# ryancinsight/imaginary

Hardware: AMD Instinct MI355X
Metric: images/sec (4K RGB->1080p Lanczos3 batch) + achieved HBM GB/s, 1/2/4/8 GPUs (higher is better)
Workload: dtype u8; 1 GPU; C2: batched 3840x2160x3 -> 1920x1080x3 Lanczos3 reduce (bimg /resize?width=1920&height=1080), corner sampling convention (PARITY_ASSUMPTIONS.md row 1), k_reduce2x2; batch_per_gpu=256, global_batch=256, parallelism=dp1 (independent shards)

## Files before the change

### imaginary_amd/csrc/k_reduce.hip

```cpp
#include <hip/hip_runtime.h>

#include <algorithm>
#include <cmath>
#include <cstdlib>
#include <vector>

#include "device_common.h"

namespace mipx {
namespace {

using namespace dev;

constexpr int kR = 12;
template <int WIDE, int TIGHT = 0>
struct R2T {
    static constexpr int kThreads = 128 << WIDE;
    static constexpr int kPitch = WIDE == 2 ? 544 : WIDE == 1 ? (TIGHT ? 264 : 288) : 160;
};

template <int B, int WIDE = 0, int TIGHT = 0>
struct R2 {
    static constexpr int kThreads = R2T<WIDE, TIGHT>::kThreads;
    static constexpr int kPitch = R2T<WIDE, TIGHT>::kPitch;
    static constexpr int TW = B == 3 ? 80 << WIDE : WIDE == 0 ? 56 : 60 << WIDE;
    static constexpr int NPX = 2 * TW + 9;
    static constexpr int K = B == 3 ? 4 : 2;
    static constexpr int OFF0 = B == 3 ? 1 : 0;
    static constexpr int ND = (B * NPX + OFF0 + 3) / 4;
    static_assert(ND <= kThreads && ND <= kPitch, "strip too wide");
    static_assert(((TW / K) * K) == TW, "items must tile the strip");
    static_assert((B * 2 * K) % 8 == 0, "window start must be 8-byte aligned");
};

struct Reduce2Args {
    const u8 *in;
    u8 *out;
    int w, h, ow, oh;
    int n_strips, n_bands, band_rows;
    int s_base, y_base, x_end, y_end;
    long long in_img, out_img;
    float c0, c1, c3, c5, bias;
    int remap;
    int band_major;
};

typedef float f2v __attribute__((ext_vector_type(2)));
typedef float f4v __attribute__((ext_vector_type(4)));

__device__ __forceinline__ f4v cvt4_once(uint32_t v) {
    return f4v{ubyte_once<0>(v), ubyte_once<1>(v), ubyte_once<2>(v), ubyte_once<3>(v)};
}
__device__ __forceinline__ f2v lo2(f4v v) { return __builtin_shufflevector(v, v, 0, 1); }
__device__ __forceinline__ f2v hi2(f4v v) { return __builtin_shufflevector(v, v, 2, 3); }

__device__ __forceinline__ float tap7(float c0, float c1, float c3, float c5, float bias, float e, float m1,
                                      float p1, float m3, float p3, float m5, float p5) {
    float acc = __builtin_fmaf(c0, e, bias);
    acc = __builtin_fmaf(c1, m1 + p1, acc);
    acc = __builtin_fmaf(c3, m3 + p3, acc);
    return __builtin_fmaf(c5, m5 + p5, acc);
}
__device__ __forceinline__ f2v tap7v(f2v c0, f2v c1, f2v c3, f2v c5, f2v bias, f2v e, f2v m1, f2v p1, f2v m3,
                                     f2v p3, f2v m5, f2v p5) {
    f2v acc = __builtin_elementwise_fma(c0, e, bias);
    acc = __builtin_elementwise_fma(c1, m1 + p1, acc);
    acc = __builtin_elementwise_fma(c3, m3 + p3, acc);
    return __builtin_elementwise_fma(c5, m5 + p5, acc);
}
__device__ __forceinline__ uint32_t pack4b(float a, float b, float c, float d) {
    uint32_t v = __builtin_amdgcn_cvt_pk_u8_f32(a, 0, 0u);
    v = __builtin_amdgcn_cvt_pk_u8_f32(b, 1, v);
    v = __builtin_amdgcn_cvt_pk_u8_f32(c, 2, v);
    return __builtin_amdgcn_cvt_pk_u8_f32(d, 3, v);
}

template <int B, int R, bool PF, bool PK, bool MEM, int LAUX, bool NTS, int WIDE, int TIGHT>
__device__ __forceinline__ void reduce2_tile(const Reduce2Args &a, int img, int strip, int band,
                                             uint32_t *lds) {
    using G = R2<B, WIDE, TIGHT>;
    constexpr int kThreads = G::kThreads, kPitch = G::kPitch;
    constexpr int TW = G::TW, K = G::K;
    const int tid = threadIdx.x;
    const int x0 = (a.s_base + strip) * TW;
    const int row_bytes = a.w * B;
    const int px0 = 2 * x0 - 5;
    const int base = (B * px0) & ~3;
    const int byte0 = base + 4 * tid;
    const bool vlane = tid < G::ND && byte0 >= 0 && byte0 + 4 <= row_bytes;
    const __amdgpu_buffer_rsrc_t rsrc = __builtin_amdgcn_make_buffer_rsrc(
        const_cast<u8 *>(a.in + img * a.in_img), 0, static_cast<int>(a.in_img), 0x00020000);
    const uint32_t voff = vlane ? static_cast<uint32_t>(byte0) : 0x80000000u;
    const int y0 = a.y_base + band * a.band_rows;
    const int y1 = min(y0 + a.band_rows, a.y_end);
    const float c0 = a.c0, c1 = a.c1, c3 = a.c3, c5 = a.c5, bias = a.bias;
    const int nl = px0 < 0 ? -px0 : 0;
    const int x_last = min(x0 + TW, a.x_end) - 1;
    const int fr = a.w - px0;
    const int fr_end = min(2 * x_last + 5 - px0, G::NPX - 1);
    const int nr = fr_end >= fr ? fr_end - fr + 1 : 0;
    const bool edge = nl > 0 || nr > 0;

    auto load_row = [&](int r) -> uint32_t {
        r = clampi(r, 0, a.h - 1);
        return static_cast<uint32_t>(__builtin_amdgcn_raw_buffer_load_b32(rsrc, voff, r * row_bytes, LAUX));
    };

    f4v ring[6];
    ring[3] = cvt4_once(load_row(2 * (y0 - 3) + 1));
    ring[4] = cvt4_once(load_row(2 * (y0 - 2) + 1));
    ring[5] = cvt4_once(load_row(2 * (y0 - 1) + 1));
    ring[0] = cvt4_once(load_row(2 * y0 + 1));
    ring[1] = cvt4_once(load_row(2 * (y0 + 1) + 1));
    ring[2] = f4v{0.f, 0.f, 0.f, 0.f};

    uint32_t odd[R], even[R];
    if (PF) {
#pragma unroll
        for (int u = 0; u < R; ++u) {
            odd[u] = load_row(2 * (y0 + u + 2) + 1);
            even[u] = load_row(2 * (y0 + u));
        }
    }
    int buf = 0;
    for (int yc = y0; yc < y1; yc += R, buf ^= 1) {
        uint32_t *L = lds + buf * (R * kPitch);
        if (!PF) {
#pragma unroll
            for (int u = 0; u < R; ++u) {
                odd[u] = load_row(2 * (yc + u + 2) + 1);
                even[u] = load_row(2 * (yc + u));
            }
        }
        const bool more = yc + R < y1;
#pragma unroll
        for (int u = 0; u < R; ++u) {
            uint32_t d;
            if (MEM) {
                d = odd[u] + even[u];
                if (PF && more) {
                    odd[u] = load_row(2 * (yc + R + u + 2) + 1);
                    even[u] = load_row(2 * (yc + R + u));
                }
            } else {
                ring[(u + 2) % 6] = cvt4_once(odd[u]);
                const f4v e = cvt4_once(even[u]);
                if (PF && more) {
                    odd[u] = load_row(2 * (yc + R + u + 2) + 1);
                    even[u] = load_row(2 * (yc + R + u));
                }
                const f4v m5 = ring[(u + 3) % 6], m3 = ring[(u + 4) % 6], m1 = ring[(u + 5) % 6];
                const f4v p1 = ring[u % 6], p3 = ring[(u + 1) % 6], p5 = ring[(u + 2) % 6];
                if (PK) {
                    const f2v C0 = {c0, c0}, C1 = {c1, c1}, C3 = {c3, c3}, C5 = {c5, c5}, BI = {bias, bias};
                    const f2v a = tap7v(C0, C1, C3, C5, BI, lo2(e), lo2(m1), lo2(p1), lo2(m3), lo2(p3), lo2(m5),
                                        lo2(p5));
                    const f2v b = tap7v(C0, C1, C3, C5, BI, hi2(e), hi2(m1), hi2(p1), hi2(m3), hi2(p3), hi2(m5),
                                        hi2(p5));
                    d = pack4b(a.x, a.y, b.x, b.y);
                } else {
                    d = pack4b(tap7(c0, c1, c3, c5, bias, e.x, m1.x, p1.x, m3.x, p3.x, m5.x, p5.x),
                               tap7(c0, c1, c3, c5, bias, e.y, m1.y, p1.y, m3.y, p3.y, m5.y, p5.y),
                               tap7(c0, c1, c3, c5, bias, e.z, m1.z, p1.z, m3.z, p3.z, m5.z, p5.z),
                               tap7(c0, c1, c3, c5, bias, e.w, m1.w, p1.w, m3.w, p3.w, m5.w, p5.w));
                }
            }
            if (G::ND >= kThreads || tid < G::ND) L[u * kPitch + tid] = d;
        }
        if (edge) {
            __syncthreads();
            u8 *Lb = reinterpret_cast<u8 *>(L);
            const int nfill = nl + nr;
            for (int i = tid; i < R * nfill * B; i += kThreads) {
                const int u = i / (nfill * B);
                const int rem = i - u * nfill * B;
                const int f = rem / B, c = rem - f * B;
                const int dst = f < nl ? f : fr + (f - nl);
                const int srcp = f < nl ? nl : fr - 1;
                Lb[u * kPitch * 4 + B * dst + G::OFF0 + c] = Lb[u * kPitch * 4 + B * srcp + G::OFF0 + c];
            }
        }
        __syncthreads();
        constexpr int items_per_row = TW / K;
        for (int it = tid; it < R * items_per_row; it += kThreads) {
            const int u = it / items_per_row;
            const int j = it - u * items_per_row;
            const int x = x0 + K * j;
            const int y = yc + u;
            if (y >= a.y_end || x >= a.x_end) continue;
            const uint32_t *row = L + u * kPitch;
            constexpr int W0 = (B * 2 * K) / 4;
            uint32_t win[13];
            if (B == 3) {
                const uint2 *r2 = reinterpret_cast<const uint2 *>(row + W0 * j);
#pragma unroll
                for (int q = 0; q < 6; ++q) {
                    const uint2 dd = r2[q];
                    win[2 * q] = dd.x;
                    win[2 * q + 1] = dd.y;
                }
                win[12] = row[W0 * j + 12];
            } else {
                const uint4 *r4 = reinterpret_cast<const uint4 *>(row + W0 * j);
#pragma unroll
                for (int q = 0; q < 3; ++q) {
                    const uint4 dd = r4[q];
                    win[4 * q] = dd.x, win[4 * q + 1] = dd.y, win[4 * q + 2] = dd.z, win[4 * q + 3] = dd.w;
                }
                win[12] = row[W0 * j + 12];
            }
            float o[K][B];
            if (MEM) {
#pragma unroll
                for (int k = 0; k < K; ++k)
#pragma unroll
                    for (int c = 0; c < B; ++c) o[k][c] = __uint_as_float(win[(k * B + c) % 13] & 0x437f0000u);
            } else
#pragma unroll
            for (int c = 0; c < B; ++c) {
                float px[2 * K + 9];
#pragma unroll
                for (int t = 0; t < 2 * K + 9; ++t) {
                    const int lb = B * t + c + G::OFF0;
                    const uint32_t dd = win[lb >> 2];
                    switch (lb & 3) {
                        case 0: px[t] = ubyte_once<0>(dd); break;
                        case 1: px[t] = ubyte_once<1>(dd); break;
                        case 2: px[t] = ubyte_once<2>(dd); break;
                        default: px[t] = ubyte_once<3>(dd); break;
                    }
                }
#pragma unroll
                for (int k = 0; k < K; ++k) {
                    const int m = 2 * k + 5;
                    o[k][c] = tap7(c0, c1, c3, c5, bias, px[m], px[m - 1], px[m + 1], px[m - 3], px[m + 3],
                                   px[m - 5], px[m + 5]);
                }
            }
            u8 *q = a.out + img * a.out_img + (static_cast<size_t>(y) * a.ow + x) * B;
            const bool full = x + K <= a.ow;
            if (B == 3) {
                const uint32_t d0 = pack4b(o[0][0], o[0][1], o[0][2], o[1][0]);
                const uint32_t d1 = pack4b(o[1][1], o[1][2], o[2][0], o[2][1]);
                const uint32_t d2 = pack4b(o[2][2], o[3][0], o[3][1], o[3][2]);
                if (full && (reinterpret_cast<uintptr_t>(q) & 3u) == 0) {
                    if (NTS) {
                        typedef uint32_t u3v __attribute__((ext_vector_type(3)));
                        __builtin_nontemporal_store(u3v{d0, d1, d2}, reinterpret_cast<u3v *>(q));
                    } else {
                        *reinterpret_cast<uint3 *>(q) = uint3{d0, d1, d2};
                    }
                } else {
                    const uint32_t dd[3] = {d0, d1, d2};
                    const int nb = (full ? K : a.ow - x) * B;
                    for (int i = 0; i < nb; ++i) q[i] = static_cast<u8>(dd[i >> 2] >> (8 * (i & 3)));
                }
            } else {
                const uint32_t d0 = pack4b(o[0][0], o[0][1], o[0][2], o[0][3]);
                const uint32_t d1 = pack4b(o[1][0], o[1][1], o[1][2], o[1][3]);
                uint32_t *q32 = reinterpret_cast<uint32_t *>(q);
                if (full && (reinterpret_cast<uintptr_t>(q) & 7u) == 0) {
                    *reinterpret_cast<uint2 *>(q) = uint2{d0, d1};
                } else {
                    q32[0] = d0;
                    if (full) q32[1] = d1;
                }
            }
        }
    }
}


template <int B, int VAR>
__global__ void __launch_bounds__(R2T<(VAR & 128) ? 2 : (VAR & 64) ? 1 : 0>::kThreads) k_reduce2x2(Reduce2Args a) {
    constexpr int WIDE = (VAR & 128) ? 2 : (VAR & 64) ? 1 : 0;
    constexpr int TIGHT = (VAR & 256) ? 1 : 0;
    constexpr int kPitch = R2T<WIDE, TIGHT>::kPitch;
    constexpr int R = (VAR & 1) ? 6 : 12;
    constexpr bool PF = (VAR & 2) != 0;
    constexpr bool PK = (VAR & 4) != 0;
    constexpr bool MEM = (VAR & 8) != 0;
    constexpr int LAUX = (VAR & 16) ? 2 : 0;
    constexpr bool NTS = (VAR & 32) != 0;
    __shared__ uint32_t lds[2 * R * kPitch];
    const uint32_t t = a.remap ? xcd_remap(blockIdx.x, gridDim.x) : blockIdx.x;
    int strip, band, img;
    if (a.band_major) {
        band = t % a.n_bands;
        const int rest = t / a.n_bands;
        strip = rest % a.n_strips;
        img = rest / a.n_strips;
    } else {
        strip = t % a.n_strips;
        const int rest = t / a.n_strips;
        band = rest % a.n_bands;
        img = rest / a.n_bands;
    }
    reduce2_tile<B, R, PF, PK, MEM, LAUX, NTS, WIDE, TIGHT>(a, img, strip, band, lds);
}


}

int reducev_launch(const u8 *in, u8 *out, int n, int w, int h, int b, double vshrink, hipStream_t st) {
    SepSpec spec;
    if (!sep_spec_reduce(vshrink, &spec)) return MIPX_EDEVICE;
    SepWindow win{};
    win.bands = b;
    win.in_pitch = w * b;
    win.in_base = 0;
    win.in_img = img_bytes(w, h, b);
    win.in_len = h;
    win.o0 = 0;
    win.out_w = w;
    win.out_h = out_size_reduce(h, vshrink);
    return vpass_launch(in, out, n, spec, win, st);
}

int reduceh_launch(const u8 *in, u8 *out, int n, int w, int h, int b, double hshrink, hipStream_t st) {
    SepSpec spec;
    if (!sep_spec_reduce(hshrink, &spec)) return MIPX_EDEVICE;
    SepWindow win{};
    win.bands = b;
    win.in_pitch = w * b;
    win.in_base = 0;
    win.in_img = img_bytes(w, h, b);
    win.in_len = w;
    win.o0 = 0;
    win.out_w = out_size_reduce(w, hshrink);
    win.out_h = h;
    return hpass_launch(in, out, n, spec, win, st);
}

int reduce_one_launch(const u8 *in, u8 *out, int n, int w, int h, int b, double hs, double vs, int ox0, int oy0,
                      int ow, int oh, hipStream_t st) {
    const char *ef = tune_env("MIPX_RSTRIP");
    const bool strip_first = ef && *ef == '1';
    if (strip_first) {
        const int se = reduce_strip_launch(in, out, n, w, h, b, hs, vs, ox0, oy0, ow, oh, st);
        if (se != MIPX_EUNSUPPORTED) return se;
    }
    const char *ec = tune_env("MIPX_RCOL");
    if (!(ec && *ec == '0')) {
        const int ce = reduce_col_launch(in, out, n, w, h, b, hs, vs, ox0, oy0, ow, oh, st);
        if (ce != MIPX_EUNSUPPORTED) return ce;
    }
    const int me = reduce_mfma_launch(in, out, n, w, h, b, hs, vs, ox0, oy0, ow, oh, st);
    if (me != MIPX_EUNSUPPORTED) return me;
    if (!strip_first) {
        const int se = reduce_strip_launch(in, out, n, w, h, b, hs, vs, ox0, oy0, ow, oh, st);
        if (se != MIPX_EUNSUPPORTED) return se;
    }
    return reduce_fused_launch(in, out, n, w, h, b, hs, vs, ox0, oy0, ow, oh, st);
}

int reduce_window_launch(const u8 *in, u8 *out, int n, int w, int h, int b, double hs, double vs, int left,
                         int top, int ow, int oh, void *ws, size_t ws_bytes, hipStream_t st) {
    const int rw = hs > 1.0 ? out_size_reduce(w, hs) : w;
    const int rh = vs > 1.0 ? out_size_reduce(h, vs) : h;
    if (left < 0 || top < 0 || ow <= 0 || oh <= 0 || left + ow > rw || top + oh > rh) return MIPX_EINVAL;
    const long long in_img = img_bytes(w, h, b);
    SepSpec sv, sh;
    if (vs > 1.0 && !sep_spec_reduce(vs, &sv)) return MIPX_EDEVICE;
    if (hs > 1.0 && !sep_spec_reduce(hs, &sh)) return MIPX_EDEVICE;
    if (vs > 1.0 && hs > 1.0) {
        const int fe = reduce_one_launch(in, out, n, w, h, b, hs, vs, left, top, ow, oh, st);
        if (fe != MIPX_EUNSUPPORTED) return fe;
        const size_t need = align_up(static_cast<size_t>(n) * w * oh * b);
        if (!ws || ws_bytes < need) return MIPX_EINVAL;
        u8 *tmp = static_cast<u8 *>(ws);
        const SepWindow v{b, w * b, 0, in_img, h, top, w, oh};
        int e = vpass_launch(in, tmp, n, sv, v, st);
        if (e) return e;
        const SepWindow hw{b, w * b, 0, img_bytes(w, oh, b), w, left, ow, oh};
        return hpass_launch(tmp, out, n, sh, hw, st);
    }
    if (vs > 1.0) {
        const SepWindow v{b, w * b, static_cast<long long>(left) * b, in_img, h, top, ow, oh};
        return vpass_launch(in, out, n, sv, v, st);
    }
    if (hs > 1.0) {
        const SepWindow hw{b, w * b, static_cast<long long>(top) * w * b, in_img, w, left, ow, oh};
        return hpass_launch(in, out, n, sh, hw, st);
    }
    return extract_launch(in, out, n, w, h, b, left, top, ow, oh, st);
}

bool reduce2_taps(float c[4]) {
    std::vector<int> t;
    reduce_table(2.0, t);
    const int n = reduce_points(2.0);
    if (n != 13) return false;
    const int *r = t.data();
    static const int zero[] = {1, 3, 7, 9, 11, 12};
    for (int z : zero)
        if (r[z] != 0) return false;
    if (r[4] != r[6] || r[2] != r[8] || r[0] != r[10]) return false;
    c[0] = static_cast<float>(r[5]);
    c[1] = static_cast<float>(r[4]);
    c[2] = static_cast<float>(r[2]);
    c[3] = static_cast<float>(r[0]);
    return true;
}

bool reduce2c_taps(float t[6]) {
    std::vector<int> tab;
    reduce_table(2.0, tab);
    const int n = reduce_points(2.0);
    if (n != 13) return false;
    const int *r = tab.data() + 64 * n;
    if (r[12] != 0) return false;
    for (int i = 0; i < 6; ++i) {
        if (r[i] != r[11 - i]) return false;
        t[i] = static_cast<float>(r[i]);
    }
    return true;
}


bool reduce2_eligible(const u8 *in, int w, int h, int b, double hs, double vs) {
    if (hs != 2.0 || vs != 2.0) return false;
    const char *e2 = tune_env("MIPX_REDUCE2");
    if (e2 && *e2 == '0') return false;
    if (b != 3 && b != 4) return false;
    if ((w * b) % 4 != 0 || (reinterpret_cast<uintptr_t>(in) % 4) != 0) return false;
    if (w < 8 || h < 8) return false;
    if (reduce_centre()) {
        static const bool centre_ok = [] { float t[6]; return reduce2c_taps(t); }();
        return centre_ok;
    }
    static const bool shape_ok = [] { float c[4]; return reduce2_taps(c); }();
    return shape_ok;
}

constexpr int kR2Default = 66;
int reduce2_variant() {
    const char *e = tune_env("MIPX_R2_VARIANT");
    if (!e || !*e) return kR2Default;
    const int v = std::atoi(e);
    switch (v) {
        case 66: return v;
        default: return kR2Default;
    }
}

int reduce2_launch(const u8 *in, u8 *out, int n, int w, int h, int b, hipStream_t st) {
    return reduce2_window_launch(in, out, n, w, h, b, 0, 0, out_size_reduce(w, 2.0), out_size_reduce(h, 2.0), st);
}

int reduce2_window_launch(const u8 *in, u8 *out, int n, int w, int h, int b, int x0, int y0, int x1, int y1,
                          hipStream_t st) {
    if (reduce_centre()) {
        float tf[6];
        if (!reduce2c_taps(tf)) return MIPX_EINVAL;
        int taps[12];
        for (int i = 0; i < 6; ++i) taps[i] = taps[11 - i] = static_cast<int>(tf[i]);
        return reduce2m_window_launch(in, out, n, w, h, b, x0, y0, x1, y1, taps, st);
    }
    float c[4];
    if (!reduce2_taps(c)) return MIPX_EINVAL;
    Reduce2Args a{};
    a.in = in;
    a.out = out;
    a.w = w;
    a.h = h;
    a.ow = out_size_reduce(w, 2.0);
    a.oh = out_size_reduce(h, 2.0);
    if (x0 < 0 || y0 < 0 || x1 > a.ow || y1 > a.oh || x0 >= x1 || y0 >= y1) return MIPX_EINVAL;
    const int var = reduce2_variant();
    const int wl = (var & 128) ? 2 : (var & 64) ? 1 : 0;
    const int tw = b == 3 ? (wl == 2 ? R2<3, 2>::TW : wl == 1 ? R2<3, 1>::TW : R2<3>::TW)
                          : (wl == 2 ? R2<4, 2>::TW : wl == 1 ? R2<4, 1>::TW : R2<4>::TW);
    a.s_base = x0 / tw;
    a.x_end = x1;
    a.y_base = y0 / kR * kR;
    a.y_end = y1;
    a.n_strips = (x1 + tw - 1) / tw - a.s_base;
    const int chunks = (y1 - a.y_base + kR - 1) / kR;
    const char *eb = tune_env("MIPX_R2_BAND");
    const int cpb = (eb && *eb) ? std::max(1, std::atoi(eb)) : 2;
    const int chunks_per_band = std::max(1, std::min(chunks, cpb));
    a.band_rows = chunks_per_band * kR;
    a.n_bands = (y1 - a.y_base + a.band_rows - 1) / a.band_rows;
    a.in_img = img_bytes(w, h, b);
    a.out_img = img_bytes(a.ow, a.oh, b);
    a.c0 = c[0] / 4096.0f;
    a.c1 = c[1] / 4096.0f;
    a.c3 = c[2] / 4096.0f;
    a.c5 = c[3] / 4096.0f;
    a.bias = 1.0f / 8192.0f;
    const char *er = tune_env("MIPX_R2_REMAP");
    a.remap = (er && *er) ? std::atoi(er) : 1;
    const char *eo = tune_env("MIPX_R2_ORDER");
    a.band_major = (eo && *eo) ? std::atoi(eo) : 0;
    const long long tiles = static_cast<long long>(a.n_strips) * a.n_bands * n;
    if (tiles > 0x7fffffffLL) return MIPX_EINVAL;
    dim3 grid(static_cast<unsigned>(tiles));
#define MIPX_R2(V)                                                                                      \
    case V: {                                                                                           \
        const dim3 blk(R2T<(V & 128) ? 2 : (V & 64) ? 1 : 0>::kThreads);                                                   \
        if (b == 3) hipLaunchKernelGGL((k_reduce2x2<3, V>), grid, blk, 0, st, a);                       \
        else hipLaunchKernelGGL((k_reduce2x2<4, V>), grid, blk, 0, st, a);                              \
        break;                                                                                          \
    }
    switch (var) {
        MIPX_R2(66)
        default: return MIPX_EINVAL;
    }
#undef MIPX_R2
    return launch_check("k_reduce2x2");
}


}
```

Measured before the change: 171,800 images/sec.

## Add one-pass reduce2x2 body with register-ring vertical pass over whole band

Introduces a one-pass kernel body for the default variant 66. It loads the rows for a band of up to two 12-row chunks into registers and computes the vertical 7-tap filter through a rolling ring of converted rows. The result is written once to LDS, followed by a single barrier and the horizontal pass. The previous chunked loop body remains available as variant 578 (selected via MIPX_R2_BAND). The goal is to cut per-chunk barriers and loop overhead by issuing more loads up front, at the cost of higher register pressure and dropping the non-temporal-store and other variant options from the default path.

```diff
diff --git a/imaginary_amd/csrc/k_reduce.hip b/imaginary_amd/csrc/k_reduce.hip
--- a/imaginary_amd/csrc/k_reduce.hip
+++ b/imaginary_amd/csrc/k_reduce.hip
@@ -73,6 +73,90 @@
     v = __builtin_amdgcn_cvt_pk_u8_f32(b, 1, v);
     v = __builtin_amdgcn_cvt_pk_u8_f32(c, 2, v);
     return __builtin_amdgcn_cvt_pk_u8_f32(d, 3, v);
+}
+
+template <int B, int WIDE, int TIGHT, bool MEM, bool NTS>
+__device__ __forceinline__ void reduce2_hitem(const Reduce2Args &a, int img, const uint32_t *row, int j, int x,
+                                              int y, float c0, float c1, float c3, float c5, float bias) {
+    using G = R2<B, WIDE, TIGHT>;
+    constexpr int K = G::K;
+    constexpr int W0 = (B * 2 * K) / 4;
+    uint32_t win[13];
+    if (B == 3) {
+        const uint2 *r2 = reinterpret_cast<const uint2 *>(row + W0 * j);
+#pragma unroll
+        for (int q = 0; q < 6; ++q) {
+            const uint2 dd = r2[q];
+            win[2 * q] = dd.x;
+            win[2 * q + 1] = dd.y;
+        }
+        win[12] = row[W0 * j + 12];
+    } else {
+        const uint4 *r4 = reinterpret_cast<const uint4 *>(row + W0 * j);
+#pragma unroll
+        for (int q = 0; q < 3; ++q) {
+            const uint4 dd = r4[q];
+            win[4 * q] = dd.x, win[4 * q + 1] = dd.y, win[4 * q + 2] = dd.z, win[4 * q + 3] = dd.w;
+        }
+        win[12] = row[W0 * j + 12];
+    }
+    float o[K][B];
+    if (MEM) {
+#pragma unroll
+        for (int k = 0; k < K; ++k)
+#pragma unroll
+            for (int c = 0; c < B; ++c) o[k][c] = __uint_as_float(win[(k * B + c) % 13] & 0x437f0000u);
+    } else
+#pragma unroll
+    for (int c = 0; c < B; ++c) {
+        float px[2 * K + 9];
+#pragma unroll
+        for (int t = 0; t < 2 * K + 9; ++t) {
+            const int lb = B * t + c + G::OFF0;
+            const uint32_t dd = win[lb >> 2];
+            switch (lb & 3) {
+                case 0: px[t] = ubyte_once<0>(dd); break;
+                case 1: px[t] = ubyte_once<1>(dd); break;
+                case 2: px[t] = ubyte_once<2>(dd); break;
+                default: px[t] = ubyte_once<3>(dd); break;
+            }
+        }
+#pragma unroll
+        for (int k = 0; k < K; ++k) {
+            const int m = 2 * k + 5;
+            o[k][c] = tap7(c0, c1, c3, c5, bias, px[m], px[m - 1], px[m + 1], px[m - 3], px[m + 3], px[m - 5],
+                           px[m + 5]);
+        }
+    }
+    u8 *q = a.out + img * a.out_img + (static_cast<size_t>(y) * a.ow + x) * B;
+    const bool full = x + K <= a.ow;
+    if (B == 3) {
+        const uint32_t d0 = pack4b(o[0][0], o[0][1], o[0][2], o[1][0]);
+        const uint32_t d1 = pack4b(o[1][1], o[1][2], o[2][0], o[2][1]);
+        const uint32_t d2 = pack4b(o[2][2], o[3][0], o[3][1], o[3][2]);
+        if (full && (reinterpret_cast<uintptr_t>(q) & 3u) == 0) {
+            if (NTS) {
+                typedef uint32_t u3v __attribute__((ext_vector_type(3)));
+                __builtin_nontemporal_store(u3v{d0, d1, d2}, reinterpret_cast<u3v *>(q));
+            } else {
+                *reinterpret_cast<uint3 *>(q) = uint3{d0, d1, d2};
+            }
+        } else {
+            const uint32_t dd[3] = {d0, d1, d2};
+            const int nb = (full ? K : a.ow - x) * B;
+            for (int i = 0; i < nb; ++i) q[i] = static_cast<u8>(dd[i >> 2] >> (8 * (i & 3)));
+        }
+    } else {
+        const uint32_t d0 = pack4b(o[0][0], o[0][1], o[0][2], o[0][3]);
+        const uint32_t d1 = pack4b(o[1][0], o[1][1], o[1][2], o[1][3]);
+        uint32_t *q32 = reinterpret_cast<uint32_t *>(q);
+        if (full && (reinterpret_cast<uintptr_t>(q) & 7u) == 0) {
+            *reinterpret_cast<uint2 *>(q) = uint2{d0, d1};
+        } else {
+            q32[0] = d0;
+            if (full) q32[1] = d1;
+        }
+    }
 }
 
 template <int B, int R, bool PF, bool PK, bool MEM, int LAUX, bool NTS, int WIDE, int TIGHT>
@@ -188,85 +272,104 @@
             const int x = x0 + K * j;
             const int y = yc + u;
             if (y >= a.y_end || x >= a.x_end) continue;
-            const uint32_t *row = L + u * kPitch;
-            constexpr int W0 = (B * 2 * K) / 4;
-            uint32_t win[13];
-            if (B == 3) {
-                const uint2 *r2 = reinterpret_cast<const uint2 *>(row + W0 * j);
-#pragma unroll
-                for (int q = 0; q < 6; ++q) {
-                    const uint2 dd = r2[q];
-                    win[2 * q] = dd.x;
-                    win[2 * q + 1] = dd.y;
-                }
-                win[12] = row[W0 * j + 12];
-            } else {
-                const uint4 *r4 = reinterpret_cast<const uint4 *>(row + W0 * j);
-#pragma unroll
-                for (int q = 0; q < 3; ++q) {
-                    const uint4 dd = r4[q];
-                    win[4 * q] = dd.x, win[4 * q + 1] = dd.y, win[4 * q + 2] = dd.z, win[4 * q + 3] = dd.w;
-                }
-                win[12] = row[W0 * j + 12];
-            }
-            float o[K][B];
-            if (MEM) {
-#pragma unroll
-                for (int k = 0; k < K; ++k)
-#pragma unroll
-                    for (int c = 0; c < B; ++c) o[k][c] = __uint_as_float(win[(k * B + c) % 13] & 0x437f0000u);
-            } else
-#pragma unroll
-            for (int c = 0; c < B; ++c) {
-                float px[2 * K + 9];
-#pragma unroll
-                for (int t = 0; t < 2 * K + 9; ++t) {
-                    const int lb = B * t + c + G::OFF0;
-                    const uint32_t dd = win[lb >> 2];
-                    switch (lb & 3) {
-                        case 0: px[t] = ubyte_once<0>(dd); break;
-                        case 1: px[t] = ubyte_once<1>(dd); break;
-                        case 2: px[t] = ubyte_once<2>(dd); break;
-                        default: px[t] = ubyte_once<3>(dd); break;
-                    }
-                }
-#pragma unroll
-                for (int k = 0; k < K; ++k) {
-                    const int m = 2 * k + 5;
-                    o[k][c] = tap7(c0, c1, c3, c5, bias, px[m], px[m - 1], px[m + 1], px[m - 3], px[m + 3],
-                                   px[m - 5], px[m + 5]);
-                }
-            }
-            u8 *q = a.out + img * a.out_img + (static_cast<size_t>(y) * a.ow + x) * B;
-            const bool full = x + K <= a.ow;
-            if (B == 3) {
-                const uint32_t d0 = pack4b(o[0][0], o[0][1], o[0][2], o[1][0]);
-                const uint32_t d1 = pack4b(o[1][1], o[1][2], o[2][0], o[2][1]);
-                const uint32_t d2 = pack4b(o[2][2], o[3][0], o[3][1], o[3][2]);
-                if (full && (reinterpret_cast<uintptr_t>(q) & 3u) == 0) {
-                    if (NTS) {
-                        typedef uint32_t u3v __attribute__((ext_vector_type(3)));
-                        __builtin_nontemporal_store(u3v{d0, d1, d2}, reinterpret_cast<u3v *>(q));
-                    } else {
-                        *reinterpret_cast<uint3 *>(q) = uint3{d0, d1, d2};
-                    }
-                } else {
-                    const uint32_t dd[3] = {d0, d1, d2};
-                    const int nb = (full ? K : a.ow - x) * B;
-                    for (int i = 0; i < nb; ++i) q[i] = static_cast<u8>(dd[i >> 2] >> (8 * (i & 3)));
-                }
-            } else {
-                const uint32_t d0 = pack4b(o[0][0], o[0][1], o[0][2], o[0][3]);
-                const uint32_t d1 = pack4b(o[1][0], o[1][1], o[1][2], o[1][3]);
-                uint32_t *q32 = reinterpret_cast<uint32_t *>(q);
-                if (full && (reinterpret_cast<uintptr_t>(q) & 7u) == 0) {
-                    *reinterpret_cast<uint2 *>(q) = uint2{d0, d1};
-                } else {
-                    q32[0] = d0;
-                    if (full) q32[1] = d1;
-                }
-            }
-        }
+            reduce2_hitem<B, WIDE, TIGHT, MEM, NTS>(a, img, L + u * kPitch, j, x, y, c0, c1, c3, c5, bias);
+        }
+    }
+}
+
+template <int NR, int ND, int kThreads, int kPitch, class LoadRow>
+__device__ __forceinline__ void reduce2_vpass(const LoadRow &load_row, int y0, int tid, float c0, float c1,
+                                              float c3, float c5, float bias, uint32_t *L) {
+    constexpr int R = kR;
+    static_assert(NR == R || NR == 2 * R, "one or two chunks");
+    uint32_t r5[5], odd[R], even[R];
+#pragma unroll
+    for (int k = 0; k < 5; ++k) r5[k] = load_row(2 * (y0 - 3 + k) + 1);
+#pragma unroll
+    for (int u = 0; u < R; ++u) {
+        odd[u] = load_row(2 * (y0 + u + 2) + 1);
+        even[u] = load_row(2 * (y0 + u));
+    }
+    f4v ring[6];
+    ring[3] = cvt4_once(r5[0]);
+    ring[4] = cvt4_once(r5[1]);
+    ring[5] = cvt4_once(r5[2]);
+    ring[0] = cvt4_once(r5[3]);
+    ring[1] = cvt4_once(r5[4]);
+    ring[2] = f4v{0.f, 0.f, 0.f, 0.f};
+#pragma unroll
+    for (int u = 0; u < NR; ++u) {
+        const int s = u % R;
+        ring[(u + 2) % 6] = cvt4_once(odd[s]);
+        const f4v e = cvt4_once(even[s]);
+        if (u + R < NR) {
+            odd[s] = load_row(2 * (y0 + R + u + 2) + 1);
+            even[s] = load_row(2 * (y0 + R + u));
+        }
+        const f4v m5 = ring[(u + 3) % 6], m3 = ring[(u + 4) % 6], m1 = ring[(u + 5) % 6];
+        const f4v p1 = ring[u % 6], p3 = ring[(u + 1) % 6], p5 = ring[(u + 2) % 6];
+        const uint32_t d = pack4b(tap7(c0, c1, c3, c5, bias, e.x, m1.x, p1.x, m3.x, p3.x, m5.x, p5.x),
+                                  tap7(c0, c1, c3, c5, bias, e.y, m1.y, p1.y, m3.y, p3.y, m5.y, p5.y),
+                                  tap7(c0, c1, c3, c5, bias, e.z, m1.z, p1.z, m3.z, p3.z, m5.z, p5.z),
+                                  tap7(c0, c1, c3, c5, bias, e.w, m1.w, p1.w, m3.w, p3.w, m5.w, p5.w));
+        if (ND >= kThreads || tid < ND) L[u * kPitch + tid] = d;
+    }
+}
+
+template <int B, int WIDE, int TIGHT>
+__device__ __forceinline__ void reduce2_onepass(const Reduce2Args &a, int img, int strip, int band,
+                                                uint32_t *lds) {
+    using G = R2<B, WIDE, TIGHT>;
+    constexpr int kThreads = G::kThreads, kPitch = G::kPitch;
+    constexpr int TW = G::TW, K = G::K;
+    const int tid = threadIdx.x;
+    const int x0 = (a.s_base + strip) * TW;
+    const int row_bytes = a.w * B;
+    const int px0 = 2 * x0 - 5;
+    const int base = (B * px0) & ~3;
+    const int byte0 = base + 4 * tid;
+    const bool vlane = tid < G::ND && byte0 >= 0 && byte0 + 4 <= row_bytes;
+    const __amdgpu_buffer_rsrc_t rsrc = __builtin_amdgcn_make_buffer_rsrc(
+        const_cast<u8 *>(a.in + img * a.in_img), 0, static_cast<int>(a.in_img), 0x00020000);
+    const uint32_t voff = vlane ? static_cast<uint32_t>(byte0) : 0x80000000u;
+    const int y0 = a.y_base + band * a.band_rows;
+    const int y1 = min(y0 + a.band_rows, a.y_end);
+    const int rows = y1 - y0;
+    const float c0 = a.c0, c1 = a.c1, c3 = a.c3, c5 = a.c5, bias = a.bias;
+    const int nl = px0 < 0 ? -px0 : 0;
+    const int x_last = min(x0 + TW, a.x_end) - 1;
+    const int fr = a.w - px0;
+    const int fr_end = min(2 * x_last + 5 - px0, G::NPX - 1);
+    const int nr = fr_end >= fr ? fr_end - fr + 1 : 0;
+
+    auto load_row = [&](int r) -> uint32_t {
+        r = clampi(r, 0, a.h - 1);
+        return static_cast<uint32_t>(__builtin_amdgcn_raw_buffer_load_b32(rsrc, voff, r * row_bytes, 0));
+    };
+    if (rows > kR) reduce2_vpass<2 * kR, G::ND, kThreads, kPitch>(load_row, y0, tid, c0, c1, c3, c5, bias, lds);
+    else reduce2_vpass<kR, G::ND, kThreads, kPitch>(load_row, y0, tid, c0, c1, c3, c5, bias, lds);
+    if (nl > 0 || nr > 0) {
+        __syncthreads();
+        u8 *Lb = reinterpret_cast<u8 *>(lds);
+        const int nfill = nl + nr;
+        for (int i = tid; i < rows * nfill * B; i += kThreads) {
+            const int u = i / (nfill * B);
+            const int rem = i - u * nfill * B;
+            const int f = rem / B, c = rem - f * B;
+            const int dst = f < nl ? f : fr + (f - nl);
+            const int srcp = f < nl ? nl : fr - 1;
+            Lb[u * kPitch * 4 + B * dst + G::OFF0 + c] = Lb[u * kPitch * 4 + B * srcp + G::OFF0 + c];
+        }
+    }
+    __syncthreads();
+    constexpr int items_per_row = TW / K;
+    for (int it = tid; it < rows * items_per_row; it += kThreads) {
+        const int u = it / items_per_row;
+        const int j = it - u * items_per_row;
+        const int x = x0 + K * j;
+        const int y = y0 + u;
+        if (x >= a.x_end) continue;
+        reduce2_hitem<B, WIDE, TIGHT, false, false>(a, img, lds + u * kPitch, j, x, y, c0, c1, c3, c5, bias);
     }
 }
 
@@ -296,7 +399,12 @@
         band = rest % a.n_bands;
         img = rest / a.n_bands;
     }
-    reduce2_tile<B, R, PF, PK, MEM, LAUX, NTS, WIDE, TIGHT>(a, img, strip, band, lds);
+    if constexpr ((VAR & 512) != 0) {
+        reduce2_tile<B, R, PF, PK, MEM, LAUX, NTS, WIDE, TIGHT>(a, img, strip, band, lds);
+    } else {
+        static_assert(R == kR && PF && !PK && !MEM && LAUX == 0 && !NTS, "the one-pass body has one build");
+        reduce2_onepass<B, WIDE, TIGHT>(a, img, strip, band, lds);
+    }
 }
 
 
@@ -434,12 +542,16 @@
 }
 
 constexpr int kR2Default = 66;
+constexpr int kR2Loop = kR2Default | 512;
 int reduce2_variant() {
+    const char *eb = tune_env("MIPX_R2_BAND");
+    if (eb && *eb) return kR2Loop;
     const char *e = tune_env("MIPX_R2_VARIANT");
     if (!e || !*e) return kR2Default;
     const int v = std::atoi(e);
     switch (v) {
-        case 66: return v;
+        case kR2Default:
+        case kR2Loop: return v;
         default: return kR2Default;
     }
 }
@@ -505,6 +617,7 @@
     }
     switch (var) {
         MIPX_R2(66)
+        MIPX_R2(578)
         default: return MIPX_EINVAL;
     }
 #undef MIPX_R2
```

Measured after the change: 174,900 images/sec, median of 6. 1.8% higher.
